# Bhumbra/probayes

Hardware: AMD Instinct MI355X
Metric: MH chain-steps/sec (whole node), 10-dim model, 65 536 chains, 1/2/4/8 GPU (higher is better)
Workload: dtype f64; 1 GPU; cfg2: 10-dim diagonal-Gaussian random-walk MH, 65536 chains/GPU, full trace every step; chains_per_gpu=65536, dim=10, trace=True, steps_per_launch=250, parallelism=chain-sharded x1

## Files before the change

probayes_amd/csrc/pbh_engine.hip:

```cpp
#include <cmath>
#include <cstdarg>
#include <cstdio>
#include <cstdlib>
#include <cstring>
#include <string>
#include <algorithm>
#include <atomic>
#include <chrono>
#include <map>
#include <mutex>
#include <unordered_map>
#include <vector>

#include "pbh_engine_state.h"
#include "pbh_expr_host.h"
#include "pbh_device.h"

using pbh::KArgs;
using pbh::check_ptr;
using pbh::dalloc;
using pbh::dfree;
using pbh::dretire;
using pbh::fail;
using pbh::srv_stop;
// ... 113 lines not shown
  if (err != hipSuccess) {
    *p = nullptr;
    return fail(PBH_ERR_HIP, "hipMalloc(%zu bytes) failed: %s", bytes, hipGetErrorString(err));
  }
  std::lock_guard<std::mutex> lk(c.mu);
  c.live.emplace(*p, bytes);
  return PBH_OK;
}

namespace {

int upload(double *&dst, const std::vector<double> &h, hipStream_t s) {
  int rc = dalloc(dst, h.size() ? h.size() : 1);
  if (rc) return rc;
  if (h.size())
    HIP_TRY(hipMemcpyAsync(dst, h.data(), h.size() * sizeof(double),
                           hipMemcpyHostToDevice, s));
  HIP_TRY(hipStreamSynchronize(s));
  return PBH_OK;
}

size_t pack(std::vector<double> &blk, const double *a, int64_t n) {
  const size_t o = blk.size();
  for (int64_t i = 0; i < n; ++i) blk.push_back(a[i]);
  return o;
}

__global__ void chains_to_dim_major(const double *init, double *x, int64_t n, int32_t d) {
  const int64_t i = (int64_t)blockIdx.x * blockDim.x + threadIdx.x;
  if (i < n * d) {
    const int64_t c = i / d, k = i - c * d;
    x[k * n + c] = init[i];
  }
}

__global__ void nacc_to_f64(const int64_t *nacc, double *out, int64_t n) {
  const int64_t i = (int64_t)blockIdx.x * blockDim.x + threadIdx.x;
  if (i < n) out[i] = (double)nacc[i];
}

void free_trace(pbh_engine *e) {
  dfree(e->tx); dfree(e->tlp); dfree(e->tpx); dfree(e->tpp); dfree(e->ts);
  dfree(e->tacc);
  e->cap = 0;
}

}

namespace {
using srv_clk = std::chrono::steady_clock;

bool srv_kernel_ended(pbh_engine *e) { return hipStreamQuery(e->stream) == hipSuccess; }

int32_t srv_first_pending(const pbh_engine *e, uint32_t seq, int32_t from) {
  for (int32_t w = from; w < e->srv_wgs; ++w)
    if (__atomic_load_n(&e->srv_done[w].seq, __ATOMIC_ACQUIRE) != seq) return w;
  return e->srv_wgs;
}
bool srv_all_done(const pbh_engine *e, uint32_t seq) {
  return srv_first_pending(e, seq, 0) == e->srv_wgs;
}

int srv_wait(pbh_engine *e, uint32_t seq, bool ok_if_ended) {
  const auto t0 = srv_clk::now();
  int32_t w = 0;
  for (uint64_t it = 1;; ++it) {
    w = srv_first_pending(e, seq, w);
    if (w == e->srv_wgs) return PBH_OK;
    if ((it & 4095) == 0) {
      const auto el = srv_clk::now() - t0;
      if (el > std::chrono::milliseconds(1) && srv_kernel_ended(e)) {
        if (srv_all_done(e, seq) || ok_if_ended) return PBH_OK;
        e->srv_active = false;
        e->srv_pending = 0;
        (void)hipStreamSynchronize(e->stream);
        (void)hipGetLastError();
        e->state_lost = true;
        return fail(PBH_ERR_HIP, "sampling server ended before command %u completed "
                    "(chain state lost: restore a checkpoint or init the chains)", seq);
      }
      if (el > std::chrono::seconds(120)) {
        e->state_lost = true;
        return fail(PBH_ERR_HIP, "sampling server: command %u not completed in 120 s", seq);
      }
    }
  }
}

int srv_settle(pbh_engine *e) {
  if (!e->srv_pending) return PBH_OK;
  const int rc = srv_wait(e, e->srv_pending, false);
  e->srv_pending = 0;
  return rc;
}

void srv_write(pbh_engine *e, uint32_t n, uint64_t arg, uint32_t q) {
  pbh::SrvCmd *cmd = (e->srv_mode & 1) ? e->srv_wmail : e->srv_cmd;
  cmd->n = n;
  cmd->arg = arg;
  __atomic_store_n(&cmd->seq, q, __ATOMIC_RELEASE);
  if (e->srv_mode & 1) __builtin_ia32_sfence();
}

int srv_alloc_fine(pbh_engine *e) {
  hipError_t err = hipExtMallocWithFlags((void **)&e->srv_mail, sizeof(pbh::SrvCmd),
                                         hipDeviceMallocFinegrained);
  if (err != hipSuccess) {
    e->srv_mail = nullptr;
    return fail(PBH_ERR_HIP, "server mailbox: %s", hipGetErrorString(err));
  }
  e->srv_mail_fine = true;
  hipPointerAttribute_t at{};
  err = hipPointerGetAttributes(&at, e->srv_mail);
  e->srv_wmail = static_cast<pbh::SrvCmd *>(err == hipSuccess ? at.hostPointer : nullptr);
  if (!e->srv_wmail) {
    dfree(e->srv_mail);
    return fail(PBH_ERR_UNSUPPORTED, "server mailbox: no host mapping");
  }
  return PBH_OK;
}

int srv_probe_direct(pbh_engine *e) {
  dfree(e->srv_mail);
  if (const int rc = srv_alloc_fine(e)) return rc;
  const uint32_t pat[4] = {0x5eed1234u, 0x0badf00du, 0x600df00du, 0xfeedfaceu};
// ... 8 lines not shown
    e->srv_wmail = nullptr;
    return fail(PBH_ERR_UNSUPPORTED, "server mailbox: host stores not seen by the device");
  }
  return PBH_OK;
}

int srv_launch(pbh_engine *e, pbh::KArgs k) {
  int32_t wgs = 0;
  hipError_t err = pbh::launch_mh_server(k, e->stream, &wgs, true);
  if (err != hipSuccess) return fail(PBH_ERR_UNSUPPORTED, "no resident server form");
  if (!e->srv_cmd) {
    err = hipHostMalloc((void **)&e->srv_cmd, sizeof(pbh::SrvCmd), hipHostMallocCoherent);
    if (err != hipSuccess) {
      e->srv_cmd = nullptr;
      return fail(PBH_ERR_HIP, "server command block: %s", hipGetErrorString(err));
    }
  }
  if (e->srv_done_len < wgs) {
    if (e->srv_done) (void)hipHostFree(e->srv_done);
    e->srv_done = nullptr;
    e->srv_done_len = 0;
    err = hipHostMalloc((void **)&e->srv_done, (size_t)wgs * sizeof(pbh::SrvDone),
                        hipHostMallocCoherent);
    if (err != hipSuccess) {
      e->srv_done = nullptr;
      return fail(PBH_ERR_HIP, "server completion words: %s", hipGetErrorString(err));
    }
    e->srv_done_len = wgs;
  }
  if (!e->srv_probed) {
    e->srv_probed = true;
    if ((e->srv_mode & 1) && srv_probe_direct(e) != PBH_OK) e->srv_mode &= ~1;
  }
  const bool direct = (e->srv_mode & 1) != 0;
  if (e->srv_mail && direct != e->srv_mail_fine) dfree(e->srv_mail);
  if (!e->srv_mail) {
    if (direct) {
      if (const int rc = srv_alloc_fine(e)) return rc;
    } else {
      err = hipMalloc((void **)&e->srv_mail, sizeof(pbh::SrvCmd));
      if (err != hipSuccess) {
        e->srv_mail = nullptr;
        return fail(PBH_ERR_HIP, "server mailbox: %s", hipGetErrorString(err));
      }
      e->srv_mail_fine = false;
      e->srv_wmail = nullptr;
    }
  }
  HIP_TRY(hipMemsetAsync(e->srv_mail, 0, sizeof(pbh::SrvCmd), e->stream));
  if (direct) HIP_TRY(hipStreamSynchronize(e->stream));
  std::memset(e->srv_done, 0, (size_t)wgs * sizeof(pbh::SrvDone));
  std::memset(e->srv_cmd, 0, sizeof(pbh::SrvCmd));
  std::atomic_thread_fence(std::memory_order_seq_cst);
  e->srv_seq = 0;
  void *dcmd = nullptr, *ddone = nullptr;
  HIP_TRY(hipHostGetDevicePointer(&dcmd, e->srv_cmd, 0));
  HIP_TRY(hipHostGetDevicePointer(&ddone, e->srv_done, 0));
  k.srv_cmd = dcmd;
  k.srv_done = ddone;
  k.srv_mail = e->srv_mail;
  k.srv_mode = e->srv_mode;
  k.srv_idle = e->srv_idle_ms * 100000;
  err = pbh::launch_mh_server(k, e->stream, &wgs, false);
  if (err != hipSuccess) return fail(PBH_ERR_HIP, "server launch: %s", hipGetErrorString(err));
  e->srv_wgs = wgs;
  e->srv_active = true;
  e->srv_last = srv_clk::now();
  ++e->srv_launches;
  return PBH_OK;
}

struct Fair { int32_t fair, rel; };
Fair launch_fair(const pbh_engine *e, int64_t m) {
  return m <= 64 ? Fair{e->fair_short, 1} : Fair{e->fair, e->fair_rel};
}

bool srv_takes(const pbh_engine *e, int64_t n_steps) {
  return n_steps <= (1 << 30) && e->g + n_steps < (int64_t(1) << 47) &&
         !(e->collect & PBH_COLLECT_MOMENTS) && e->has_pred && e->cap > 0 && e->thin == 1 &&
         e->g - e->rec_base >= 0 && e->g + n_steps - e->rec_base <= e->cap &&
         pbh::pair_index_hi_const(e->g, n_steps);
}

void srv_submit(pbh_engine *e, int64_t n_steps) {
  const uint32_t q = ++e->srv_seq;
  const Fair f = launch_fair(e, n_steps);
  srv_write(e, (uint32_t)n_steps,
            pbh::srv_arg(e->g, (uint32_t)f.fair, (uint32_t)f.rel, pbh::kSrvRun, q), q);
  e->srv_pending = q;
  e->srv_last = srv_clk::now();
  e->g += n_steps;
  e->has_pred = true;
  e->mom_steps += n_steps;
  e->timed = true;
  e->srv_timed = true;
  e->last_launches = 1;
  ++e->srv_commands;
}

class TimedRegion {
  pbh_engine *e;
  pbh::LaunchEvents &lev;

 public:
  explicit TimedRegion(pbh_engine *eng) : e(eng), lev(pbh::launch_events()) {}
  ~TimedRegion() { lev = {}; }
  int open() {
    e->srv_timed = false;
    if (e->event_markers) HIP_TRY(hipEventRecord(e->ev0, e->stream));
    lev = {e->event_markers ? nullptr : e->ev0, nullptr};
    return PBH_OK;
  }
  void last_dispatch() {
    if (!e->event_markers) lev.stop = e->ev1;
  }
  int close() {
    lev = {};
    if (e->event_markers) HIP_TRY(hipEventRecord(e->ev1, e->stream));
    return PBH_OK;
  }
};

int run_closed(pbh_engine *e, int64_t n_steps, int64_t launches) {
  e->mom_steps += n_steps;
  e->timed = n_steps > 0;
  e->last_launches = launches;
  return PBH_OK;
}
}

int pbh::srv_stop(pbh_engine *e) {
  if (!e->srv_active) return PBH_OK;
  HIP_TRY(hipSetDevice(e->device));
  int rc = srv_settle(e);
  if (!srv_kernel_ended(e)) {
    const uint32_t q = ++e->srv_seq;
    srv_write(e, 0u, pbh::srv_arg(0, 0u, 0u, pbh::kSrvExit, q), q);
    const int rc2 = srv_wait(e, q, true);
    if (!rc) rc = rc2;
  }
  const hipError_t err = hipStreamSynchronize(e->stream);
  e->srv_active = false;
  if (!rc && err != hipSuccess)
    rc = fail(PBH_ERR_HIP, "sampling server exit: %s", hipGetErrorString(err));
  return rc;
}

extern "C" {

const char *pbh_last_error(void) { return g_err.c_str(); }

int pbh_abi_version(void) { return PBH_ABI_VERSION; }
int pbh_abi_revision(void) { return PBH_ABI_REVISION; }

int pbh_device_count(int *count) {
  if (check_ptr(count, "count")) return PBH_ERR_ARG;
  HIP_TRY(hipGetDeviceCount(count));
  return PBH_OK;
}

int pbh_create(int device, pbh_engine **out) {
  if (check_ptr(out, "out")) return PBH_ERR_ARG;
  *out = nullptr;
  int nd = 0;
  HIP_TRY(hipGetDeviceCount(&nd));
  if (device < 0 || device >= nd)
    return fail(PBH_ERR_ARG, "device %d out of range (%d devices)", device, nd);
  HIP_TRY(hipSetDevice(device));
  {
    const char *sf = std::getenv("PBH_SPIN_FLAG");
    if (sf && sf[0] == '1') {
      const hipError_t before = hipPeekAtLastError();
      if (hipSetDeviceFlags(hipDeviceScheduleSpin) != hipSuccess && before == hipSuccess)
        (void)hipGetLastError();
    }
  }
  pbh_engine *e = new pbh_engine();
  e->device = device;
  if (const char *np = std::getenv("PBH_NO_PAIR")) e->pair_enabled = np[0] != '1';
  if (const char *gm = std::getenv("PBH_GIBBS_MFMA")) e->gibbs_mfma = gm[0] != '0';
  if (const char *gf = std::getenv("PBH_GIBBS_FAST")) e->gibbs_fast = gf[0] != '0';
  if (const char *gl = std::getenv("PBH_GIBBS_LANES")) e->gibbs_lanes = std::atoi(gl);
  if (const char *ml = std::getenv("PBH_GMM_LANES")) e->gmm_lanes = std::atoi(ml);
  if (const char *sy = std::getenv("PBH_SYNC")) {
    e->spin_sync = std::strcmp(sy, "block") != 0;
    e->sync_event = std::strcmp(sy, "event") == 0;
  }
  if (const char *em = std::getenv("PBH_EVENT_MARKERS")) e->event_markers = std::atoi(em) != 0;
  if (const char *gf = std::getenv("PBH_GMM_FULL")) e->gmm_full = std::atoi(gf) != 0;
  if (const char *pf = std::getenv("PBH_PAIR_FULL")) e->pair_full = std::atoi(pf) != 0;
// ... 1107 lines not shown
  if (err == hipSuccess)
    err = hipMemcpy(out, dout, (size_t)n_steps * n * sizeof(double), hipMemcpyDeviceToHost);
  dfree(dout);
  if (err != hipSuccess) return fail(PBH_ERR_HIP, "pbh_legacy_draws: %s", hipGetErrorString(err));
  return PBH_OK;
}

int pbh_sync(pbh_engine *e) {
  if (check_ptr(e, "engine")) return PBH_ERR_ARG;
  if (e->srv_active) return srv_settle(e);
  HIP_TRY(hipSetDevice(e->device));
  if (e->spin_sync) {
    const auto t0 = std::chrono::steady_clock::now();
    hipError_t q;
    if (e->sync_event && e->timed) {
      while ((q = hipEventQuery(e->ev1)) == hipErrorNotReady) {
        if (std::chrono::steady_clock::now() - t0 > std::chrono::microseconds(2000)) break;
      }
    }
    while ((q = hipStreamQuery(e->stream)) == hipErrorNotReady) {
      if (std::chrono::steady_clock::now() - t0 > std::chrono::microseconds(2000)) {
        q = hipStreamSynchronize(e->stream);
        break;
      }
    }
    HIP_TRY(q);
  } else {
    HIP_TRY(hipStreamSynchronize(e->stream));
  }
  return PBH_OK;
}

int pbh_set_collect(pbh_engine *e, int32_t flags) {
  if (check_ptr(e, "engine")) return PBH_ERR_ARG;
  if (flags & ~PBH_COLLECT_MOMENTS) return fail(PBH_ERR_ARG, "bad collect flags %d", flags);
  e->collect = flags;
  return PBH_OK;
}

int pbh_last_run_ms(pbh_engine *e, double *ms, int64_t *launches) {
  if (check_ptr(e, "engine") || check_ptr(ms, "ms")) return PBH_ERR_ARG;
  if (!e->timed) {
    *ms = 0.;
    if (launches) *launches = 0;
    return PBH_OK;
  }
  if (e->srv_timed) {
    if (e->srv_active && e->srv_pending) {
      const int rc = pbh_sync(e);
      if (rc) return rc;
    }
    uint64_t t0 = ~0ull, t1 = 0;
    for (int32_t w = 0; w < e->srv_wgs; ++w) {
      t0 = std::min<uint64_t>(t0, __atomic_load_n(&e->srv_done[w].t0, __ATOMIC_ACQUIRE));
      t1 = std::max<uint64_t>(t1, __atomic_load_n(&e->srv_done[w].t1, __ATOMIC_ACQUIRE));
    }
    *ms = t1 > t0 ? (double)(t1 - t0) * 1e-5 : 0.;
    if (launches) *launches = e->last_launches;
    return PBH_OK;
  }
  HIP_TRY(hipEventSynchronize(e->ev1));
  float f = 0.f;
  HIP_TRY(hipEventElapsedTime(&f, e->ev0, e->ev1));
  *ms = f;
  if (launches) *launches = e->last_launches;
  return PBH_OK;
}

int pbh_server_stop(pbh_engine *e) {
  if (check_ptr(e, "engine")) return PBH_ERR_ARG;
  SRV_STOP(e);
  return PBH_OK;
}

int pbh_server_info(pbh_engine *e, int32_t *active, int64_t *commands, int64_t *launches) {
  if (check_ptr(e, "engine")) return PBH_ERR_ARG;
  if (active) *active = e->srv_active && !srv_kernel_ended(e) ? 1 : 0;
  if (commands) *commands = e->srv_commands;
  if (launches) *launches = e->srv_launches;
  return PBH_OK;
}

int pbh_server_stamps(pbh_engine *e, int32_t cap, uint32_t *seq, uint64_t *t0,
                      uint64_t *t1, int32_t *n) {
  if (check_ptr(e, "engine") || check_ptr(n, "n")) return PBH_ERR_ARG;
  *n = e->srv_done ? e->srv_wgs : 0;
  for (int32_t w = 0; w < *n && w < cap; ++w) {
    if (seq) seq[w] = __atomic_load_n(&e->srv_done[w].seq, __ATOMIC_ACQUIRE);
    if (t0) t0[w] = __atomic_load_n(&e->srv_done[w].t0, __ATOMIC_ACQUIRE);
    if (t1) t1[w] = __atomic_load_n(&e->srv_done[w].t1, __ATOMIC_ACQUIRE);
  }
  return PBH_OK;
}

int pbh_get_state(pbh_engine *e, double *x, double *logp) {
  if (check_ptr(e, "engine")) return PBH_ERR_ARG;
  SRV_STOP(e);
  if (!e->x) return fail(PBH_ERR_STATE, "pbh_init_chains first");
  HIP_TRY(hipSetDevice(e->device));
  HIP_TRY(hipStreamSynchronize(e->stream));
  const int64_t n = e->n;
  const int d = e->d;
  if (x) {
    std::vector<double> xt((size_t)n * d);
    HIP_TRY(hipMemcpy(xt.data(), e->x, xt.size() * sizeof(double), hipMemcpyDeviceToHost));
    pbh::dim_major_to_rows(xt.data(), x, n, d);
  }
  if (logp) HIP_TRY(hipMemcpy(logp, e->lp, n * sizeof(double), hipMemcpyDeviceToHost));
  return PBH_OK;
}

int pbh_get_checkpoint(pbh_engine *e, double *x, double *lp, int64_t *step,
                       int32_t *has_pred, uint32_t *xo) {
  int rc = pbh_get_state(e, x, lp);
  if (rc) return rc;
  if (step) *step = e->g;
  if (has_pred) *has_pred = e->has_pred ? 1 : 0;
  if (xo) {
    if (e->rng != PBH_RNG_XOSHIRO)
      return fail(PBH_ERR_STATE, "no xoshiro state (rng is not XOSHIRO)");
    HIP_TRY(hipSetDevice(e->device));
    if (!e->xo_seeded) {
      HIP_TRY(pbh::launch_xo_seed(e->xo, e->n, e->off, e->seed, e->stream));
      e->xo_seeded = true;
    }
    HIP_TRY(hipStreamSynchronize(e->stream));
    HIP_TRY(hipMemcpy(xo, e->xo, (size_t)8 * e->n * sizeof(uint32_t),
                      hipMemcpyDeviceToHost));
  }
  return PBH_OK;
}

static int replace_chains(pbh_engine *e, const double *x, const double *lp, int64_t step,
                          int32_t has_pred, bool restore, const uint32_t *xo) {
  if (check_ptr(e, "engine") || check_ptr(x, "x") || check_ptr(lp, "lp"))
    return PBH_ERR_ARG;
  SRV_STOP(e);
  if (!e->x) return fail(PBH_ERR_STATE, "pbh_init_chains first");
  if (step < 0) return fail(PBH_ERR_ARG, "step index must be >= 0");
  if (restore && e->rng == PBH_RNG_XOSHIRO && !xo)
    return fail(PBH_ERR_ARG, "XOSHIRO needs the generator state xo");
  const int64_t n = e->n;
  HIP_TRY(hipSetDevice(e->device));
// ... 314 lines not shown
```

probayes_amd/csrc/pbh_engine_state.h:

```cpp
#pragma once
#include <hip/hip_runtime.h>
#include <rccl/rccl.h>

#include <chrono>
#include <vector>

#include "../../include/pbhip.h"
#include "pbh_kernels.h"

struct pbh_engine {
  int device = 0;
  hipStream_t stream = nullptr;
  hipEvent_t ev0 = nullptr, ev1 = nullptr;
  unsigned ev_flags = 0;
  bool has_model = false, has_prop = false, has_gibbs = false;
  int d = 0;
  pbh::KArgs k{};
  double *dmodel = nullptr, *dprop = nullptr, *dgibbs = nullptr;
  std::vector<int32_t> draw_order;
  int64_t n = 0, off = 0;
  double *x = nullptr, *lp = nullptr;
  bool has_pred = false;
  int64_t g = 0;
  int32_t rng = PBH_RNG_PHILOX;
// ... 15 lines not shown
  double *ess_tot = nullptr;
  size_t thr_alloc = 0;
  int64_t thr_steps = 0;
  int32_t *mt_pos = nullptr, *mt_has = nullptr, *mt_order = nullptr;
  double *mt_gauss = nullptr;
  bool mt_stale = false;
  int64_t cap = 0;
  int32_t thin = 1, debug = 0;
  int64_t rec_base = 0;
  double *tx = nullptr, *tlp = nullptr, *tpx = nullptr, *tpp = nullptr,
         *ts = nullptr;
  uint64_t *tacc = nullptr;
  int32_t collect = PBH_COLLECT_MOMENTS;
  double *msum = nullptr, *msq = nullptr;
  int64_t *nacc = nullptr;
  int64_t mom_steps = 0;
  double *bm64 = nullptr;
  double *lgtab = nullptr;
  double *ess = nullptr;
  int32_t *ess_list = nullptr;
  size_t ess_list_len = 0;
  double *stage = nullptr;
  size_t stage_len = 0;
  unsigned char *scratch = nullptr;
  size_t scratch_bytes = 0;
  bool spin_sync = true;
  bool sync_event = false;
  bool gmm_full = true;
  bool pair_full = true;
  int ess_fft = 2;
  bool iid_full = true;
  int fair = 11;
  int pair_wg = 512;
  int fair_short = 10;
  int fair_rel = 0;
  bool event_markers = true;
  bool pair_enabled = true;
  bool gibbs_mfma = true;
  bool gibbs_fast = true;
  int gibbs_lanes = 0;
  int gmm_lanes = 4;
  std::vector<double> mvn_mean, mvn_U;
  double mvn_const = 0.;
  double *gq = nullptr;
  double *lx = nullptr;
  bool lx_valid = false;
  bool gq_valid = false;
  bool timed = false;
  int64_t last_launches = 0;
  bool srv_enabled = false;
  bool srv_active = false;
  bool srv_timed = false;
  uint32_t srv_seq = 0, srv_pending = 0;
  int32_t srv_wgs = 0;
  int64_t srv_idle_ms = 1000;
  pbh::SrvCmd *srv_cmd = nullptr;
  pbh::SrvDone *srv_done = nullptr;
  pbh::SrvCmd *srv_mail = nullptr;
  int32_t srv_done_len = 0;
  int32_t srv_mode = 1;
  bool srv_probed = false;
  bool srv_mail_fine = false;
  pbh::SrvCmd *srv_wmail = nullptr;
  std::chrono::steady_clock::time_point srv_last{};
  bool state_lost = false;
  int64_t srv_commands = 0, srv_launches = 0;
  ncclComm_t comm = nullptr;
  int32_t rank = 0, world = 1;
  double *gather_send = nullptr, *gather_recv = nullptr, *scalar = nullptr;
};

namespace pbh {

int fail(int code, const char *fmt, ...);

inline int check_ptr(const void *p, const char *name) {
  return p ? PBH_OK : fail(PBH_ERR_ARG, "%s must not be NULL", name);
}

#define HIP_TRY(expr)                                                        \
  do {                                                                       \
    hipError_t _e = (expr);                                                  \
    if (_e != hipSuccess)                                                    \
      return pbh::fail(PBH_ERR_HIP, "%s failed: %s", #expr, hipGetErrorString(_e)); \
  } while (0)

enum class DMem { Alloc, Free, Retire };
int dmem(DMem op, void **p, size_t bytes = 0);

template <class T>
int dalloc(T *&p, size_t count) { return dmem(DMem::Alloc, (void **)&p, count * sizeof(T)); }
template <class T>
void dfree(T *&p) { (void)dmem(DMem::Free, (void **)&p); }
template <class T>
void dretire(T *&p) { (void)dmem(DMem::Retire, (void **)&p); }
template <class T>
int dgrow(T *&p, size_t &len, size_t need) {
  if (len >= need) return PBH_OK;
  len = 0;
  if (const int rc = dalloc(p, need)) return rc;
  len = need;
  return PBH_OK;
}

inline void rows_to_dim_major(const double *rows, double *dm, int64_t n, int64_t d) {
  for (int64_t c = 0; c < n; ++c)
// ... 32 lines not shown
```

probayes_amd/csrc/pbh_kernels.h:

```cpp
#pragma once
#include <hip/hip_runtime.h>
#include <hip/hip_ext.h>
#include <stdint.h>

#include "pbh_expr_words.h"

namespace pbh {

struct LaunchEvents {
  hipEvent_t start = nullptr, stop = nullptr;
};
LaunchEvents &launch_events();
bool module_launch();
hipFunction_t kernel_function(const void *kernel);

template <typename F, typename... Args>
inline void pbh_launch(F kernel, const dim3 &grid, const dim3 &block,
                       size_t shm, hipStream_t st, Args... args) {
  LaunchEvents &ev = launch_events();
  if (ev.start || ev.stop) {
    (void)hipExtLaunchKernelGGL(kernel, grid, block, (uint32_t)shm, st, ev.start,
                                ev.stop, 0u, args...);
  } else if (const hipFunction_t fn = module_launch()
                 ? kernel_function(reinterpret_cast<const void *>(kernel)) : nullptr) {
    void *params[] = {reinterpret_cast<void *>(&args)...};
    (void)hipModuleLaunchKernel(fn, grid.x, grid.y, grid.z, block.x, block.y, block.z,
                                (unsigned)shm, st, params, nullptr);
  } else {
    hipLaunchKernelGGL(kernel, grid, block, shm, st, args...);
  }
  ev.start = nullptr;
}


struct KArgs {
  int32_t d, target, pscale, scores;
  const double *ta, *tb, *tc, *te;
  int64_t tn;
  int32_t i0, i1;
  int32_t has_prior;
  const double *plo, *phi;
  uint32_t plo_incl, phi_incl;
  double prior_logp;
  uint32_t ufun;
  int32_t tran_kind, tran_sym, tran_rev;
  double tran_value, tran_scale;
  const double *tran_off;
  int32_t prop;
  const double *ploc, *pscl, *plen, *pdel;
  int32_t ploc_zero;
  double sdelta;
  const double *ptf;
  int32_t has_tfun;
  uint64_t vmode;
  uint32_t vint;
  uint32_t bnd_on, bnd_xlo, bnd_xhi;
  const double *blo, *bhi;
  const double *gmean, *gcoef, *gstdv, *gcdf;
// ... 13 lines not shown
  int32_t rng;
  uint32_t seed_lo, seed_hi;
  const double *rep;
  uint32_t *xo;
  int64_t rep_row0;
  int32_t R;
  double *tx, *tlp, *tpx, *tpp, *ts;
  uint64_t *tacc;
  int32_t thin;
  int64_t rec_base;
  int64_t rec_cap;
  int32_t debug;
  int64_t W;
  int32_t pair_ok;
  int32_t simple_acc;
  double acc_beta;
  int32_t gibbs_mfma;
  int32_t gibbs_fast;
  const double *gpp;
  const double *gmup;
  const double *gzlo, *gzhi;
  const double *gak;
  double gconst;
  double *gq;
  int32_t gq_init;
  double *lx;
  int32_t lx_init;
  int32_t gibbs_lanes;
  int32_t gmm_lanes;
  int32_t gmm_full;
  int32_t pair_full;
  int32_t iid_full;
  int32_t fair;
  int32_t pair_wg;
  int32_t fair_rel;
  void *srv_cmd;
  void *srv_done;
  void *srv_mail;
  int64_t srv_idle;
  int32_t srv_mode;
  int32_t moments;
  double *msum, *msq;
  int64_t *nacc;
  const double *bm64;
  const int32_t *ecode;
  const double *econst;
  int32_t en;
  const double *edata;
  const int32_t *eleaf;
  int32_t enobs, enpad, enleaf;
  int32_t ewide;
};
constexpr int kTargetExprData = 8;
struct alignas(16) SrvCmd {
  uint32_t seq, n;
  uint64_t arg;
};
__host__ __device__ inline uint64_t srv_arg(int64_t g0, uint32_t fair, uint32_t fair_rel,
                                            uint32_t op, uint32_t seq) {
  return ((uint64_t)g0 & 0xFFFFFFFFFFFFull) | ((uint64_t)(fair & 31u) << 48) |
         ((uint64_t)(fair_rel & 1u) << 53) | ((uint64_t)(op & 1u) << 54) |
         ((uint64_t)(seq & 0xFFu) << 56);
}
struct SrvDone {
  uint32_t seq, pad;
  uint64_t t0, t1;
  uint64_t pad2;
};
constexpr uint32_t kSrvRun = 0, kSrvExit = 1;


inline bool gibbs_fast_form(const KArgs &a) {
  return a.gibbs_fast && a.rng == 1  && !a.debug && a.d <= 16;
}

inline bool pair_index_hi_const(int64_t g0, int64_t n) {
  return n < 1 || (g0 >> 33) == ((g0 + n - 1) >> 33);
}

hipError_t launch_mh(const KArgs &a, hipStream_t s, size_t lds_bytes);
hipError_t launch_gibbs(const KArgs &a, hipStream_t s);
hipError_t launch_mh_server(const KArgs &a, hipStream_t s, int32_t *wgs, bool check);
hipError_t launch_xo_seed(uint32_t *xo, int64_t n, int64_t off, uint64_t seed,
                          hipStream_t s);
bool mh_dim_supported(int d);
hipError_t launch_mh_expr(const KArgs &a, hipStream_t s);
hipError_t launch_eval_expr(const KArgs &a, int64_t n, const double *x, double *out);
hipError_t launch_check_normals(int64_t n, const uint32_t *words, double *fast,
                                double *ref);
hipError_t launch_check_normals64(int64_t n, const uint32_t *words,
                                  const double *tab, double *fast, double *ref);
hipError_t launch_trace_stats(const double *tx, const uint64_t *tacc, int64_t n,
                              int32_t d, int64_t W, int64_t first,
                              int64_t count, double *sum, double *sumsq,
                              int64_t *nacc, hipStream_t s);
hipError_t launch_trace_expectation(const double *tx, const double *tlp,
                                    int64_t n, int32_t d, int64_t first,
                                    int64_t count, double exponent, int32_t lin,
                                    double log_npi, double *out, hipStream_t s);
hipError_t launch_trace_quantile(const double *tx, const double *tlp, int64_t n,
                                 int32_t d, int64_t first, int32_t count, int32_t nq,
                                 const double *q, int32_t weighted, int32_t lin,
                                 double log_npi, double *out, hipStream_t s);
hipError_t launch_rhat_chain(const double *tx, int64_t n, int32_t d, int64_t first,
                             int64_t count, double *stats, hipStream_t s);
hipError_t launch_rhat_cross(const double *stats, int64_t n, int32_t d, int64_t count,
                             int64_t group, double *sc, double *split_out,
                             double *nested_out, hipStream_t s);
constexpr int kSelectMaxTargets = 129;
int64_t select_scratch_words(int32_t d, int32_t nt);
int64_t select_stats_offset(int32_t d, int32_t nt);
int32_t select_passes();
hipError_t launch_select_init(uint64_t *sc, int32_t d, int32_t nt, const uint64_t *ranks,
                              uint64_t *host, hipStream_t s);
hipError_t launch_select_pass(const double *tx, int64_t n, int32_t d, int64_t first,
                              int64_t count, uint64_t *sc, int32_t nt, int32_t pass,
                              hipStream_t s);
struct RankLayout;
hipError_t launch_rank_dim(const double *tx, int64_t n, int32_t d, int32_t k, int64_t first,
                           int64_t count, const double *med, unsigned char *scratch,
                           const RankLayout &l, bool want_ranks, hipStream_t s);
struct EssLayout;
// ... 99 lines not shown
```

probayes_amd/csrc/pbh_kernels_impl.h:

```cpp
#pragma once
#include <utility>

#include "pbh_kernels.h"
#include "pbh_device.h"
#include "../../include/pbhip.h"

namespace pbh {

namespace {

constexpr int kBlock = 256;
constexpr int kPairFullBlock = 512;

__device__ __forceinline__ double cld(const double *p, int64_t i) {
  return ((const __attribute__((address_space(4))) double *)p)[i];
}

__device__ __forceinline__ double uni(double v) {
  const uint64_t u = __builtin_bit_cast(uint64_t, v);
  const uint32_t lo = __builtin_amdgcn_readfirstlane((uint32_t)u);
  const uint32_t hi = __builtin_amdgcn_readfirstlane((uint32_t)(u >> 32));
  return __builtin_bit_cast(double, (uint64_t)lo | ((uint64_t)hi << 32));
}

// ... 1214 lines not shown
              else rb[n - H] = z;
            }
          }
        };
        auto step_full = [&](int si, const double (&r)[H], uint32_t t0) {
          double xp[H];
#pragma unroll
          for (int i = 0; i < H; ++i)
            xp[i] = LOC0 ? __builtin_fma(r[i], psc[i], x[i])
                         : x[i] + __builtin_fma(r[i], psc[i], plc[i]);
          double p0 = 0., p1 = 0.;
#pragma unroll
          for (int i = 0; i < H; ++i) {
            const double u = __builtin_fma(xp[i], cb[i], -ca[i]);
            if (i & 1) p1 = __builtin_fma(u, u, p1);
            else p0 = __builtin_fma(u, u, p0);
          }
          double lo, up;
          halves_f64(p0 + p1, lo, up);
          const double lpp = (-(lo + up)) - a.ksum;
          const float eL = __builtin_amdgcn_exp2f(
              (float)__builtin_fma(lpp - lp, 1.4426950408889634, 16.0));
          const float fl = (float)t0;
          const uint64_t inp = __ballot(__builtin_fabs(lpp) <= 700.);
          const uint64_t inr = inp & inl;
          const uint64_t af = __ballot(fl <= __builtin_fmaf(eL, 0.999996f, -1.0f));
          const uint64_t rf = __ballot(fl > eL * 1.000004f);
          uint64_t accm = inr & af;
          const uint64_t needm = ~(inr & (af | rf)) & kHi;
          if (needm) {
            bool ex = false;
            if (__builtin_amdgcn_inverse_ballot_w64(needm))
              ex = pair_exact(a.seed_lo, a.seed_hi, a.log_npi, g0v + si, chain, h,
                              t0, lpp, lp);
            accm = (accm & ~needm) | (__ballot(ex) & needm);
          }
          const uint64_t mhi = accm & kHi;
          const uint64_t macc = mhi | (mhi >> 32);
#pragma unroll
          for (int i = 0; i < H; ++i) x[i] = sel_f64(macc, x[i], xp[i]);
          lp = sel_f64(macc, lp, lpp);
          inl = (inl & ~macc) | (inp & macc);
          double *row = a.tx + rec * D * a.n;
#pragma unroll
          for (int i = 0; i < H; ++i) st_buf(row, boff, i * bstride, x[i]);
          st_buf_n(a.tlp + rec * a.n, lpbytes, lpoff, lp);
          st_buf32_n(reinterpret_cast<uint32_t *>(a.tacc + rec * a.W), abytes, aoff,
                     (uint32_t)(mhi >> 32));
          ++rec;
        };
        using I0 = std::integral_constant<int, 0>;
        using IA = std::integral_constant<int, QA>;
        using IH = std::integral_constant<int, H>;
        auto run_block = [&]() {
          if (g0v & 1) {
            constexpr int QB = 3 * (H / 2) / 4;
            uint32_t w[4 * NB];
            philox_from(g0v >> 1, w, std::integral_constant<int, QB>{});
            normals(w, std::integral_constant<int, H / 2>{}, IH{}, cA, cB);
            __builtin_amdgcn_s_waitcnt(0);
            step_full(0, cB, w[3 * H] & 0xFFFFu);
            s = 1;
          }
          if (s + 1 < nsv) {
            uint32_t w[4 * NB];
            philox((g0v + s) >> 1, w);
            normals(w, I0{}, IH{}, cA, cB);
            ctA = w[3 * H] >> 16;
            ctB = w[3 * H] & 0xFFFFu;
            if (s == 0) __builtin_amdgcn_s_waitcnt(0);
            PBH_PHASE(2);
            const uint32_t slot = fairv ? simd_wave_slot() : 0u;
            const uint64_t tfair0 =
                fair_relv ? __builtin_amdgcn_s_memrealtime() : 0ull;
            for (; s + 3 < nsv; s += 2) {
              if (fairv) {
                const int64_t el = (int64_t)(__builtin_amdgcn_s_memrealtime() - tfair0);
                fair_prio((uint32_t)((el > 0 ? (uint64_t)el : 0ull) >> fairv) + slot);
              }
              PBH_PHASE_Q(s >> 1, nsv >> 1);
              uint32_t nw[4 * NB];
              double nA[H], nB[H];
              philox(((g0v + s) >> 1) + 1, nw);
              step_full(s, cA, ctA);
              normals(nw, I0{}, IA{}, nA, nB);
              step_full(s + 1, cB, ctB);
              normals(nw, IA{}, IH{}, nA, nB);
  #pragma unroll
              for (int i = 0; i < H; ++i) {
                cA[i] = nA[i];
                cB[i] = nB[i];
              }
              ctA = nw[3 * H] >> 16;
              ctB = nw[3 * H] & 0xFFFFu;
            }
            step_full(s, cA, ctA);
            step_full(s + 1, cB, ctB);
            s += 2;
          }
          if (s < nsv) {
            uint32_t w[4 * NB];
            philox((g0v + s) >> 1, w);
            normals(w, I0{}, IA{}, cA, cB);
            if (s == 0) __builtin_amdgcn_s_waitcnt(0);
            step_full(s, cA, w[3 * H] >> 16);
          }
        };
        if constexpr (SRV) {
          __shared__ int64_t s_cmd[6];
          SrvCmd *const hcmd = reinterpret_cast<SrvCmd *>(a.srv_cmd);
          SrvCmd *const mail = reinterpret_cast<SrvCmd *>(a.srv_mail);
          SrvDone *const donep = reinterpret_cast<SrvDone *>(a.srv_done) + blockIdx.x;
          const bool poller = __builtin_amdgcn_readfirstlane((int)(threadIdx.x >> 6)) == 0;
          const bool direct = (a.srv_mode & 1) != 0;
          const bool relay = blockIdx.x == 0 && !direct;
          uint32_t seen = 0u;
          for (;;) {
            if (poller) {
              const uint64_t tw = __builtin_amdgcn_s_memrealtime();
              const SrvCmd *src = relay ? hcmd : mail;
              uint32_t q;
              u32x4v v;
              for (;;) {
                v = ld16_sys(src);
                q = (uint32_t)__builtin_amdgcn_readfirstlane((int)v.x);
                const uint32_t chk = (uint32_t)__builtin_amdgcn_readfirstlane((int)v.w) >> 24;
                if (q != seen && chk == (q & 0xFFu)) break;
                if (__builtin_amdgcn_s_memrealtime() - tw > (uint64_t)a.srv_idle) {
                  q = 0u;
                  break;
                }
                __builtin_amdgcn_s_sleep(1);
              }
              const uint64_t tsee = __builtin_amdgcn_s_memrealtime();
              if (relay && q) st16_sys(mail, v);
              const uint32_t n = (uint32_t)__builtin_amdgcn_readfirstlane((int)v.y);
              const uint64_t arg =
                  (uint64_t)(uint32_t)__builtin_amdgcn_readfirstlane((int)v.z) |
                  ((uint64_t)(uint32_t)__builtin_amdgcn_readfirstlane((int)v.w) << 32);
              const int64_t g0 = (int64_t)(arg & 0xFFFFFFFFFFFFull);
              const uint32_t fr = (uint32_t)(arg >> 48) & 31u, frel = (uint32_t)(arg >> 53) & 1u;
              const uint32_t op = (uint32_t)(arg >> 54) & 1u;
              s_cmd[0] = q;
              s_cmd[1] = op;
              s_cmd[2] = g0;
              s_cmd[3] = n;
              s_cmd[4] = ((int64_t)frel << 32) | fr;
              s_cmd[5] = (int64_t)tsee;
            }
            __syncthreads();
            const uint32_t q = (uint32_t)__builtin_amdgcn_readfirstlane((int)s_cmd[0]);
            const uint32_t op = (uint32_t)__builtin_amdgcn_readfirstlane((int)s_cmd[1]);
            if (q == 0u || op == kSrvExit) {
              if (poller && q != 0u)
                __hip_atomic_store(&donep->seq, q, __ATOMIC_RELAXED, __HIP_MEMORY_SCOPE_SYSTEM);
              break;
            }
            const int64_t c2 = s_cmd[2], c4 = s_cmd[4];
            g0v = (int64_t)(uint32_t)__builtin_amdgcn_readfirstlane((int)(uint32_t)c2) |
                  ((int64_t)__builtin_amdgcn_readfirstlane((int)(c2 >> 32)) << 32);
            nsv = __builtin_amdgcn_readfirstlane((int)s_cmd[3]);
            fairv = __builtin_amdgcn_readfirstlane((int)(uint32_t)c4);
            fair_relv = __builtin_amdgcn_readfirstlane((int)(c4 >> 32));
            const uint64_t tseen = (uint64_t)s_cmd[5];
            s = 0;
            rec = g0v - a.rec_base;
            if ((uint32_t)((uint64_t)g0v >> 33) != pre_hi) {
              pre_hi = (uint32_t)((uint64_t)g0v >> 33);
              pre = philox_prefix<NB>(16u * (uint32_t)h, chain, pre_hi, a.seed_lo, a.seed_hi);
            }
            run_block();
            __builtin_amdgcn_s_waitcnt(0);
            __syncthreads();
            if (poller) {
              __hip_atomic_store(&donep->t0, tseen, __ATOMIC_RELAXED, __HIP_MEMORY_SCOPE_SYSTEM);
              __hip_atomic_store(&donep->t1, (uint64_t)__builtin_amdgcn_s_memrealtime(),
                                 __ATOMIC_RELAXED, __HIP_MEMORY_SCOPE_SYSTEM);
              __builtin_amdgcn_s_waitcnt(0);
              __hip_atomic_store(&donep->seq, q, __ATOMIC_RELAXED, __HIP_MEMORY_SCOPE_SYSTEM);
            }
            seen = q;
          }
        } else {
          run_block();
        }
        PBH_PHASE(3);
    } else {
      if (a.g0 & 1) {
        PD::draw(a, s_bmt, h, a.g0 >> 1, chain, cA, cB, ctA, ctB);
        step(s, cB, ctB, t1);
        ++s;
      }
      for (; s + 1 < a.n_steps; s += 2) {
        PD::draw(a, s_bmt, h, (a.g0 + s) >> 1, chain, cA, cB, ctA, ctB);
        step(s, cA, ctA, t1);
        step(s + 1, cB, ctB, t1);
      }
      if (s < a.n_steps) {
        PD::draw(a, s_bmt, h, (a.g0 + s) >> 1, chain, cA, cB, ctA, ctB);
        step(s, cA, ctA, t1);
      }
    }
  } else {
    double r[H];
    uint32_t t0 = 0, t1 = 0;
    for (int s = 0; s < a.n_steps; ++s) step(s, r, t0, t1);
  }

  if (active) {
#pragma unroll
    for (int i = 0; i < H; ++i) a.x[(k0 + i) * a.n + c] = x[i];
    if (hi) a.lp[c] = lp;
    if constexpr (mom) {
#pragma unroll
      for (int i = 0; i < H; ++i) {
        a.msum[(k0 + i) * a.n + c] += ms[i];
        a.msq[(k0 + i) * a.n + c] += mq[i];
      }
      if (hi) a.nacc[c] += nacc;
    }
    if (RNG == PBH_RNG_XOSHIRO) xo_store(a, h, c, xs);
  }
  if constexpr (FULL) {
    PBH_PHASE(4);
    PBH_PHASE_STORE(a.rep, wave, lane);
  }
}
template <int L>
__device__ __forceinline__ void gather_f64(double v, double (&all)[L]) {
  if constexpr (L == 2) {
    halves_f64(v, all[0], all[1]);
  } else {
    static_assert(L == 4, "lanes per chain: 2 or 4");
    double ev, od;
    rowpair_f64(v, ev, od);
    halves_f64(ev, all[0], all[2]);
    halves_f64(od, all[1], all[3]);
// ... 1465 lines not shown
```

Baseline: 47.90 billion chain-steps/s.

## Precompute next command's first random pair in server kernel; harden command/done records

In the persistent sampling server, after finishing a run command each workgroup precomputes the Philox normals for the next expected step pair (and the odd-step half), so the next command can start stepping without the RNG latency on its critical path. The command checksum now covers seq, n and payload, and completion records are written as two 16-byte system stores carrying a second sequence copy, so the host reads only whole records and ignores torn timestamps. This adds register pressure from the prefetched arrays and extra host-side validation logic.

```diff
diff --git a/probayes_amd/csrc/pbh_engine.hip b/probayes_amd/csrc/pbh_engine.hip
--- a/probayes_amd/csrc/pbh_engine.hip
+++ b/probayes_amd/csrc/pbh_engine.hip
@@ -189,25 +189,38 @@
 
 bool srv_kernel_ended(pbh_engine *e) { return hipStreamQuery(e->stream) == hipSuccess; }
 
-int32_t srv_first_pending(const pbh_engine *e, uint32_t seq, int32_t from) {
+bool srv_done_whole(const pbh::SrvDone &d, uint32_t q) {
+  return __atomic_load_n(&d.seq, __ATOMIC_ACQUIRE) == q &&
+         (uint32_t)__atomic_load_n(&d.seq2, __ATOMIC_ACQUIRE) == q;
+}
+bool srv_record_of_run(const pbh_engine *e, const pbh::SrvDone &d) {
+  const uint32_t q = __atomic_load_n(&d.seq, __ATOMIC_ACQUIRE);
+  return e->srv_run_seq != 0 &&
+         (uint32_t)__atomic_load_n(&d.seq2, __ATOMIC_ACQUIRE) == e->srv_run_seq &&
+         (q == e->srv_run_seq || (e->srv_exit_seq != 0 && q == e->srv_exit_seq));
+}
+
+int32_t srv_first_pending(const pbh_engine *e, uint32_t seq, int32_t from, bool run) {
   for (int32_t w = from; w < e->srv_wgs; ++w)
-    if (__atomic_load_n(&e->srv_done[w].seq, __ATOMIC_ACQUIRE) != seq) return w;
+    if (run ? !srv_done_whole(e->srv_done[w], seq)
+            : __atomic_load_n(&e->srv_done[w].seq, __ATOMIC_ACQUIRE) != seq)
+      return w;
   return e->srv_wgs;
 }
-bool srv_all_done(const pbh_engine *e, uint32_t seq) {
-  return srv_first_pending(e, seq, 0) == e->srv_wgs;
+bool srv_all_done(const pbh_engine *e, uint32_t seq, bool run) {
+  return srv_first_pending(e, seq, 0, run) == e->srv_wgs;
 }
 
 int srv_wait(pbh_engine *e, uint32_t seq, bool ok_if_ended) {
   const auto t0 = srv_clk::now();
   int32_t w = 0;
   for (uint64_t it = 1;; ++it) {
-    w = srv_first_pending(e, seq, w);
+    w = srv_first_pending(e, seq, w, !ok_if_ended);
     if (w == e->srv_wgs) return PBH_OK;
     if ((it & 4095) == 0) {
       const auto el = srv_clk::now() - t0;
       if (el > std::chrono::milliseconds(1) && srv_kernel_ended(e)) {
-        if (srv_all_done(e, seq) || ok_if_ended) return PBH_OK;
+        if (ok_if_ended || srv_all_done(e, seq, true)) return PBH_OK;
         e->srv_active = false;
         e->srv_pending = 0;
         (void)hipStreamSynchronize(e->stream);
@@ -322,7 +335,7 @@
   std::memset(e->srv_done, 0, (size_t)wgs * sizeof(pbh::SrvDone));
   std::memset(e->srv_cmd, 0, sizeof(pbh::SrvCmd));
   std::atomic_thread_fence(std::memory_order_seq_cst);
-  e->srv_seq = 0;
+  e->srv_seq = e->srv_run_seq = e->srv_exit_seq = 0;
   void *dcmd = nullptr, *ddone = nullptr;
   HIP_TRY(hipHostGetDevicePointer(&dcmd, e->srv_cmd, 0));
   HIP_TRY(hipHostGetDevicePointer(&ddone, e->srv_done, 0));
@@ -356,8 +369,11 @@
   const uint32_t q = ++e->srv_seq;
   const Fair f = launch_fair(e, n_steps);
   srv_write(e, (uint32_t)n_steps,
-            pbh::srv_arg(e->g, (uint32_t)f.fair, (uint32_t)f.rel, pbh::kSrvRun, q), q);
+            pbh::srv_arg(e->g, (uint32_t)f.fair, (uint32_t)f.rel, pbh::kSrvRun, q,
+                         (uint32_t)n_steps), q);
   e->srv_pending = q;
+  e->srv_run_seq = q;
+  e->srv_exit_seq = 0;
   e->srv_last = srv_clk::now();
   e->g += n_steps;
   e->has_pred = true;
@@ -405,7 +421,8 @@
   int rc = srv_settle(e);
   if (!srv_kernel_ended(e)) {
     const uint32_t q = ++e->srv_seq;
-    srv_write(e, 0u, pbh::srv_arg(0, 0u, 0u, pbh::kSrvExit, q), q);
+    srv_write(e, 0u, pbh::srv_arg(0, 0u, 0u, pbh::kSrvExit, q, 0u), q);
+    e->srv_exit_seq = q;
     const int rc2 = srv_wait(e, q, true);
     if (!rc) rc = rc2;
   }
@@ -1619,6 +1636,7 @@
     }
     uint64_t t0 = ~0ull, t1 = 0;
     for (int32_t w = 0; w < e->srv_wgs; ++w) {
+      if (!srv_record_of_run(e, e->srv_done[w])) continue;
       t0 = std::min<uint64_t>(t0, __atomic_load_n(&e->srv_done[w].t0, __ATOMIC_ACQUIRE));
       t1 = std::max<uint64_t>(t1, __atomic_load_n(&e->srv_done[w].t1, __ATOMIC_ACQUIRE));
     }
@@ -1653,9 +1671,10 @@
   if (check_ptr(e, "engine") || check_ptr(n, "n")) return PBH_ERR_ARG;
   *n = e->srv_done ? e->srv_wgs : 0;
   for (int32_t w = 0; w < *n && w < cap; ++w) {
+    const bool whole = srv_record_of_run(e, e->srv_done[w]);
     if (seq) seq[w] = __atomic_load_n(&e->srv_done[w].seq, __ATOMIC_ACQUIRE);
-    if (t0) t0[w] = __atomic_load_n(&e->srv_done[w].t0, __ATOMIC_ACQUIRE);
-    if (t1) t1[w] = __atomic_load_n(&e->srv_done[w].t1, __ATOMIC_ACQUIRE);
+    if (t0) t0[w] = whole ? __atomic_load_n(&e->srv_done[w].t0, __ATOMIC_ACQUIRE) : 0;
+    if (t1) t1[w] = whole ? __atomic_load_n(&e->srv_done[w].t1, __ATOMIC_ACQUIRE) : 0;
   }
   return PBH_OK;
 }
diff --git a/probayes_amd/csrc/pbh_engine_state.h b/probayes_amd/csrc/pbh_engine_state.h
--- a/probayes_amd/csrc/pbh_engine_state.h
+++ b/probayes_amd/csrc/pbh_engine_state.h
@@ -91,6 +91,7 @@
   bool srv_active = false;
   bool srv_timed = false;
   uint32_t srv_seq = 0, srv_pending = 0;
+  uint32_t srv_run_seq = 0, srv_exit_seq = 0;
   int32_t srv_wgs = 0;
   int64_t srv_idle_ms = 1000;
   pbh::SrvCmd *srv_cmd = nullptr;
diff --git a/probayes_amd/csrc/pbh_kernels.h b/probayes_amd/csrc/pbh_kernels.h
--- a/probayes_amd/csrc/pbh_kernels.h
+++ b/probayes_amd/csrc/pbh_kernels.h
@@ -4,6 +4,7 @@
 #include <stdint.h>
 
 #include "pbh_expr_words.h"
+#include "pbh_srv_record.h"
 
 namespace pbh {
 
@@ -123,22 +124,6 @@
   int32_t ewide;
 };
 constexpr int kTargetExprData = 8;
-struct alignas(16) SrvCmd {
-  uint32_t seq, n;
-  uint64_t arg;
-};
-__host__ __device__ inline uint64_t srv_arg(int64_t g0, uint32_t fair, uint32_t fair_rel,
-                                            uint32_t op, uint32_t seq) {
-  return ((uint64_t)g0 & 0xFFFFFFFFFFFFull) | ((uint64_t)(fair & 31u) << 48) |
-         ((uint64_t)(fair_rel & 1u) << 53) | ((uint64_t)(op & 1u) << 54) |
-         ((uint64_t)(seq & 0xFFu) << 56);
-}
-struct SrvDone {
-  uint32_t seq, pad;
-  uint64_t t0, t1;
-  uint64_t pad2;
-};
-constexpr uint32_t kSrvRun = 0, kSrvExit = 1;
 
 
 inline bool gibbs_fast_form(const KArgs &a) {
diff --git a/probayes_amd/csrc/pbh_kernels_impl.h b/probayes_amd/csrc/pbh_kernels_impl.h
--- a/probayes_amd/csrc/pbh_kernels_impl.h
+++ b/probayes_amd/csrc/pbh_kernels_impl.h
@@ -1290,23 +1290,60 @@
         using I0 = std::integral_constant<int, 0>;
         using IA = std::integral_constant<int, QA>;
         using IH = std::integral_constant<int, H>;
-        auto run_block = [&]() {
+        double pA[H], pB[H];
+        uint32_t ptA = 0, ptB = 0;
+        bool pm_have = false;
+        int64_t pm_g = 0;
+        uint32_t pm_hi = 0;
+        auto make_pair = [&](int64_t P, double (&ra)[H], double (&rb)[H], uint32_t &ta,
+                             uint32_t &tb) {
+          uint32_t w[4 * NB];
+          philox(P, w);
+          normals(w, I0{}, IH{}, ra, rb);
+          ta = w[3 * H] >> 16;
+          tb = w[3 * H] & 0xFFFFu;
+        };
+        auto make_step_b = [&](int64_t P) {
+          constexpr int QB = 3 * (H / 2) / 4;
+          uint32_t w[4 * NB];
+          philox_from(P, w, std::integral_constant<int, QB>{});
+          normals(w, std::integral_constant<int, H / 2>{}, IH{}, cA, cB);
+          ctB = w[3 * H] & 0xFFFFu;
+        };
+        auto run_block = [&](const bool pm_in) -> bool {
+          const bool pm = SRV && pm_in;
+          bool pleft = pm;
           if (g0v & 1) {
-            constexpr int QB = 3 * (H / 2) / 4;
-            uint32_t w[4 * NB];
-            philox_from(g0v >> 1, w, std::integral_constant<int, QB>{});
-            normals(w, std::integral_constant<int, H / 2>{}, IH{}, cA, cB);
-            __builtin_amdgcn_s_waitcnt(0);
-            step_full(0, cB, w[3 * H] & 0xFFFFu);
+            if (pm) {
+              step_full(0, cB, ctB);
+            } else {
+              constexpr int QB = 3 * (H / 2) / 4;
+              uint32_t w[4 * NB];
+              philox_from(g0v >> 1, w, std::integral_constant<int, QB>{});
+              normals(w, std::integral_constant<int, H / 2>{}, IH{}, cA, cB);
+              __builtin_amdgcn_s_waitcnt(0);
+              step_full(0, cB, w[3 * H] & 0xFFFFu);
+            }
             s = 1;
           }
           if (s + 1 < nsv) {
-            uint32_t w[4 * NB];
-            philox((g0v + s) >> 1, w);
-            normals(w, I0{}, IH{}, cA, cB);
-            ctA = w[3 * H] >> 16;
-            ctB = w[3 * H] & 0xFFFFu;
-            if (s == 0) __builtin_amdgcn_s_waitcnt(0);
+            pleft = false;
+            if (pm) {
+#pragma unroll
+              for (int i = 0; i < H; ++i) {
+                cA[i] = pA[i];
+                cB[i] = pB[i];
+              }
+              ctA = ptA;
+              ctB = ptB;
+            } else {
+              uint32_t w[4 * NB];
+              philox((g0v + s) >> 1, w);
+              normals(w, I0{}, IH{}, cA, cB);
+              ctA = w[3 * H] >> 16;
+              ctB = w[3 * H] & 0xFFFFu;
+              if (s == 0) __builtin_amdgcn_s_waitcnt(0);
+            }
             PBH_PHASE(2);
             const uint32_t slot = fairv ? simd_wave_slot() : 0u;
             const uint64_t tfair0 =
@@ -1337,12 +1374,17 @@
             s += 2;
           }
           if (s < nsv) {
-            uint32_t w[4 * NB];
-            philox((g0v + s) >> 1, w);
-            normals(w, I0{}, IA{}, cA, cB);
-            if (s == 0) __builtin_amdgcn_s_waitcnt(0);
-            step_full(s, cA, w[3 * H] >> 16);
+            if (pleft) {
+              step_full(s, pA, ptA);
+            } else {
+              uint32_t w[4 * NB];
+              philox((g0v + s) >> 1, w);
+              normals(w, I0{}, IA{}, cA, cB);
+              if (s == 0) __builtin_amdgcn_s_waitcnt(0);
+              step_full(s, cA, w[3 * H] >> 16);
+            }
           }
+          return pleft;
         };
         if constexpr (SRV) {
           __shared__ int64_t s_cmd[6];
@@ -1362,8 +1404,12 @@
               for (;;) {
                 v = ld16_sys(src);
                 q = (uint32_t)__builtin_amdgcn_readfirstlane((int)v.x);
-                const uint32_t chk = (uint32_t)__builtin_amdgcn_readfirstlane((int)v.w) >> 24;
-                if (q != seen && chk == (q & 0xFFu)) break;
+                if (q != seen &&
+                    srv_cmd_whole(q, (uint32_t)__builtin_amdgcn_readfirstlane((int)v.y),
+                                  (uint64_t)(uint32_t)__builtin_amdgcn_readfirstlane((int)v.z) |
+                                      ((uint64_t)(uint32_t)__builtin_amdgcn_readfirstlane((int)v.w)
+                                       << 32)))
+                  break;
                 if (__builtin_amdgcn_s_memrealtime() - tw > (uint64_t)a.srv_idle) {
                   q = 0u;
                   break;
@@ -1407,20 +1453,44 @@
               pre_hi = (uint32_t)((uint64_t)g0v >> 33);
               pre = philox_prefix<NB>(16u * (uint32_t)h, chain, pre_hi, a.seed_lo, a.seed_hi);
             }
-            run_block();
+            const bool pm = __builtin_amdgcn_readfirstlane(
+                                (int)(pm_have && pm_g == g0v && pm_hi == pre_hi)) != 0;
+            const bool pleft = __builtin_amdgcn_readfirstlane((int)run_block(pm)) != 0;
             __builtin_amdgcn_s_waitcnt(0);
             __syncthreads();
             if (poller) {
-              __hip_atomic_store(&donep->t0, tseen, __ATOMIC_RELAXED, __HIP_MEMORY_SCOPE_SYSTEM);
-              __hip_atomic_store(&donep->t1, (uint64_t)__builtin_amdgcn_s_memrealtime(),
-                                 __ATOMIC_RELAXED, __HIP_MEMORY_SCOPE_SYSTEM);
-              __builtin_amdgcn_s_waitcnt(0);
-              __hip_atomic_store(&donep->seq, q, __ATOMIC_RELAXED, __HIP_MEMORY_SCOPE_SYSTEM);
+              const uint64_t tdone = __builtin_amdgcn_s_memrealtime();
+              st16_sys(&donep->seq, u32x4v{q, 0u, (uint32_t)tseen, (uint32_t)(tseen >> 32)});
+              st16_sys(&donep->t1, u32x4v{(uint32_t)tdone, (uint32_t)(tdone >> 32), q, 0u});
             }
             seen = q;
+            const int64_t gn = g0v + nsv;
+            const uint32_t gn_hi = (uint32_t)((uint64_t)gn >> 33);
+            pm_have = (uint32_t)((uint64_t)(gn + 1) >> 33) == gn_hi;
+            pm_g = gn;
+            pm_hi = gn_hi;
+            if (pm_have) {
+              if (gn_hi != pre_hi) {
+                pre_hi = gn_hi;
+                pre = philox_prefix<NB>(16u * (uint32_t)h, chain, pre_hi, a.seed_lo, a.seed_hi);
+              }
+              if (gn & 1) {
+                if (pleft) {
+#pragma unroll
+                  for (int i = 0; i < H; ++i) cB[i] = pB[i];
+                  ctB = ptB;
+                } else {
+                  make_step_b(gn >> 1);
+                }
+                make_pair((gn >> 1) + 1, pA, pB, ptA, ptB);
+              } else if (!pleft) {
+                make_pair(gn >> 1, pA, pB, ptA, ptB);
+              }
+            }
           }
         } else {
-          run_block();
+          (void)pm_have, (void)pm_g, (void)pm_hi;
+          (void)run_block(false);
         }
         PBH_PHASE(3);
     } else {
diff --git a/probayes_amd/csrc/pbh_srv_record.h b/probayes_amd/csrc/pbh_srv_record.h
--- /dev/null
+++ b/probayes_amd/csrc/pbh_srv_record.h
@@ -0,0 +1,44 @@
+#pragma once
+#include <stdint.h>
+
+#if defined(__HIPCC__)
+#define PBH_SRV_FN __host__ __device__ __forceinline__
+#else
+#define PBH_SRV_FN inline
+#endif
+
+namespace pbh {
+
+struct alignas(16) SrvCmd {
+  uint32_t seq, n;
+  uint64_t arg;
+};
+constexpr uint64_t kSrvPayloadMask = 0x00FFFFFFFFFFFFFFull;
+
+PBH_SRV_FN uint32_t srv_fold8(uint32_t v, uint32_t turn) {
+  v ^= v >> 16;
+  v = (v ^ (v >> 8)) & 0xFFu;
+  return ((v << turn) | (v >> (8u - turn))) & 0xFFu;
+}
+PBH_SRV_FN uint32_t srv_check(uint32_t seq, uint32_t n, uint64_t payload) {
+  return (seq & 0xFFu) ^ srv_fold8(n, 3u) ^ srv_fold8((uint32_t)payload, 5u) ^
+         srv_fold8((uint32_t)(payload >> 32) & 0xFFFFFFu, 6u);
+}
+PBH_SRV_FN uint64_t srv_arg(int64_t g0, uint32_t fair, uint32_t fair_rel, uint32_t op,
+                            uint32_t seq, uint32_t n) {
+  const uint64_t payload = ((uint64_t)g0 & 0xFFFFFFFFFFFFull) | ((uint64_t)(fair & 31u) << 48) |
+                           ((uint64_t)(fair_rel & 1u) << 53) | ((uint64_t)(op & 1u) << 54);
+  return payload | ((uint64_t)srv_check(seq, n, payload) << 56);
+}
+PBH_SRV_FN bool srv_cmd_whole(uint32_t seq, uint32_t n, uint64_t arg) {
+  return (uint32_t)(arg >> 56) == srv_check(seq, n, arg & kSrvPayloadMask);
+}
+
+struct SrvDone {
+  uint32_t seq, pad;
+  uint64_t t0, t1;
+  uint64_t seq2;
+};
+constexpr uint32_t kSrvRun = 0, kSrvExit = 1;
+
+}
```

After: 46.05 billion chain-steps/s. -3.9%, worse.
